# DTUComputeStatisticsAndDataAnalysis/MBPLS

Measured on NVIDIA B200. Metric: MB-PLS NIPALS fit: algorithmic HBM GB/s (n=10k, p=1M, 4 blocks, 20 LV, fp64), higher is better.
Workload: dtype f64

## Files before the change

### mbpls_b200/csrc/fused.cu

```cuda
#include "launch.cuh"
#include "../../include/mbpls_b200.h"

using namespace mbpls;

namespace {

struct FusedArgs {
  const double* Xt;
  double* Xw;
  long ld;
  int n;
  const double* u;
  const double* uu;
  const double* ts;
  const double* rden;
  const double* rden2;
  const int* split_f0;
  const int* split_f1;
  const int* split_block;
  int nsplit;
  int B;
  double* w;
  double* norm_part;
  double* Tnum;
  long ldt;
  double* P_k;
  double* pss;
  const int* done;
  int sync_mode;
};

template <int TG, int EPTC_, int CPF_, int S_>
struct Cfg {
  static constexpr int kTG = TG, EPTC = EPTC_, CPF = CPF_, S = S_;
  static constexpr int G = 512 / TG, EPT = EPTC_ * CPF_, NW = TG / 32;
  static constexpr int UC = TG * EPTC_;
};

template <int NV, int TG>
__device__ __forceinline__ void worker_sum(double (&v)[NV], double* buf, int g, int warp_in_group, int lane) {
  constexpr int NW = TG / 32;
#pragma unroll
  for (int k = 0; k < NV; ++k) v[k] = warp_sum(v[k]);
  if (lane == 0) {
#pragma unroll
    for (int k = 0; k < NV; ++k) buf[k * NW + warp_in_group] = v[k];
  }
  asm volatile("bar.sync %0, %1;" ::"r"(g + 1), "n"(TG) : "memory");
#pragma unroll
  for (int k = 0; k < NV; ++k) {
    const double2* pr = reinterpret_cast<const double2*>(buf + k * NW);
    if (NW == 2) {
      const double2 p0 = pr[0];
      v[k] = p0.x + p0.y;
    } else {
      double grp[NW >= 4 ? NW / 4 : 1];
#pragma unroll
      for (int q = 0; q < NW / 4; ++q) {
        const double2 p0 = pr[2 * q], p1 = pr[2 * q + 1];
        grp[q] = (p0.x + p0.y) + (p1.x + p1.y);
      }
      double t = grp[0];
      if (NW == 8) t = grp[0] + grp[1];
      if (NW == 16) t = (grp[0] + grp[1]) + (grp[2] + grp[3]);
      v[k] = t;
    }
  }
}

__device__ __forceinline__ unsigned atom_inc_smem(unsigned* p) {
  unsigned old;
  asm volatile("atom.relaxed.cta.shared::cta.add.u32 %0, [%1], 1;" : "=r"(old) : "r"(smem_u32(p)) : "memory");
  return old;
}
__device__ __forceinline__ unsigned atom_inc_smem_acqrel(unsigned* p) {
  unsigned old;
  asm volatile("atom.acq_rel.cta.shared::cta.add.u32 %0, [%1], 1;" : "=r"(old) : "r"(smem_u32(p)) : "memory");
  return old;
}

template <class C>
struct Smem {
  double* vec0;
  double* vec1;
  double* ring;
  uint64_t* full;
  unsigned* cnt;
  double* scratch;
  uint64_t* xbar;
  double* xval;
  __device__ Smem(unsigned char* base, long vlen, int nvec) {
    vec0 = reinterpret_cast<double*>(base);
    vec1 = vec0 + vlen;
    ring = vec0 + static_cast<size_t>(nvec) * vlen;
    full = reinterpret_cast<uint64_t*>(ring + static_cast<size_t>(C::G) * C::S * 2 * C::UC);
    cnt = reinterpret_cast<unsigned*>(full + C::G * C::S);
    scratch = reinterpret_cast<double*>(full + 2 * C::G * C::S);
    xbar = reinterpret_cast<uint64_t*>(scratch + static_cast<size_t>(C::G) * 2 * 3 * C::NW);
    xval = reinterpret_cast<double*>(xbar + 2 * C::G);
  }
  __device__ __forceinline__ double* stage(int g, int s) const { return ring + (static_cast<size_t>(g) * C::S + s) * 2 * C::UC; }
};

template <class C>
size_t fused_smem_bytes(long vlen, int nvec) {
  return static_cast<size_t>(nvec) * vlen * 8 + static_cast<size_t>(C::G) * C::S * C::UC * 16 + static_cast<size_t>(C::G) * C::S * 16 +
         static_cast<size_t>(C::G) * 2 * 3 * C::NW * 8 + static_cast<size_t>(C::G) * 32 + 64;
}

template <class C>
__device__ __forceinline__ void issue_chunk(const double* __restrict__ X, long ld, int units, int g, int s, int f, int c,
                                            const Smem<C>& sm) {
  const int nun = min(C::UC, units - c * C::UC);
  const uint32_t bytes = static_cast<uint32_t>(nun) * 16u;
  uint64_t* fb = &sm.full[g * C::S + s];
  mbar_arrive_expect_tx(fb, bytes);
  bulk_g2s(sm.stage(g, s), X + static_cast<size_t>(f) * ld + static_cast<size_t>(c) * C::UC * 2, bytes, fb);
}

template <class C>
__device__ __forceinline__ void init_sync(const Smem<C>& sm, int sync_mode) {
  if (threadIdx.x == 0) {
    for (int i = 0; i < C::G * C::S; ++i) {
      mbar_init(&sm.full[i], 1);
      if (sync_mode == 2) mbar_init(reinterpret_cast<uint64_t*>(&sm.cnt[2 * i]), C::NW);
      else sm.cnt[2 * i] = 0;
    }
    for (int i = 0; i < 2 * C::G; ++i) mbar_init(&sm.xbar[i], 1);
    fence_barrier_init();
  }
}

template <class C>
__device__ __forceinline__ void prime_ring(const double* __restrict__ X, long ld, int units, int ncf, int g, int f0, int f1,
                                           const Smem<C>& sm) {
  int f = f0, c = 0;
  for (int s = 0; s < C::S && f < f1; ++s) {
    issue_chunk<C>(X, ld, units, g, s, f, c, sm);
    if (++c == ncf) { c = 0; ++f; }
  }
}

template <class C>
__device__ __forceinline__ bool arrive_stage(int g, int s, int lane, const Smem<C>& sm, int sync_mode, uint32_t parity) {
  __syncwarp();
  if (lane != 0) return false;
  unsigned* c = &sm.cnt[2 * (g * C::S + s)];
  if (sync_mode == 2) {
    uint64_t* eb = reinterpret_cast<uint64_t*>(c);
    if (mbar_pending_count(mbar_arrive_state(eb)) != 1u) return false;
    mbar_wait(eb, parity);
    fence_proxy_async_smem();
    return true;
  }
  const unsigned old = sync_mode ? atom_inc_smem_acqrel(c) : atom_inc_smem(c);
  if (old != C::NW - 1) return false;
  *reinterpret_cast<volatile unsigned*>(c) = 0;
  if (sync_mode) fence_proxy_async_smem();
  return true;
}

template <class C>
__device__ __forceinline__ void refill_if_last(bool last, const double* __restrict__ X, long ld, int units, int ncf, int g, int s,
                                               int j, int c, int f1, const Smem<C>& sm) {
  if (last) {
    int c2 = c + C::S, f2 = j;
    while (c2 >= ncf) { c2 -= ncf; ++f2; }
    if (f2 < f1) issue_chunk<C>(X, ld, units, g, s, f2, c2, sm);
  }
}

template <class C>
__device__ __forceinline__ double pair_sum(double own, int g, int tg, uint32_t peer, int& xs, uint32_t& xp, const Smem<C>& sm) {
  uint64_t* bar = &sm.xbar[2 * g + xs];
  double* slot = &sm.xval[2 * g + xs];
  if (tg == 0) {
    mbar_arrive_expect_tx(bar, 8);
    st_async_f64(mapa_shared(smem_u32(slot), peer), own, mapa_shared(smem_u32(bar), peer));
  }
  mbar_wait(bar, (xp >> xs) & 1u);
  const double other = *reinterpret_cast<volatile double*>(slot);
  xp ^= 1u << xs;
  xs ^= 1;
  return own + other;
}

__device__ __forceinline__ double2 nan_to_zero(double2 v) {
  if (isnan(v.x)) v.x = 0.0;
  if (isnan(v.y)) v.y = 0.0;
  return v;
}

struct Geo {
  int units;
  int uoff;
  int nloc;
  int wbase;
  uint32_t peer;
  bool lead;
};
template <class C, bool CL>
__device__ __forceinline__ Geo make_geo(long ld, int n) {
  Geo ge;
  const int total = static_cast<int>(ld >> 1);
  if (CL) {
    const uint32_t r = cluster_ctarank();
    ge.units = total >> 1;
    ge.uoff = static_cast<int>(r) * ge.units;
    ge.wbase = static_cast<int>(blockIdx.x >> 1) * C::G;
    ge.peer = r ^ 1u;
    ge.lead = r == 0;
  } else {
    ge.units = total;
    ge.uoff = 0;
    ge.wbase = static_cast<int>(blockIdx.x) * C::G;
    ge.peer = 0;
    ge.lead = true;
  }
  ge.nloc = max(0, min(2 * ge.units, n - 2 * ge.uoff));
  return ge;
}

template <bool NANMODE, class C, bool CL>
__device__ __forceinline__ void fused_trip_body(const FusedArgs& a, const Smem<C>& sm, const Geo& ge) {
  const long ld = a.ld;
  const int units = ge.units;
  const int ncf = (units + C::UC - 1) / C::UC;
  const int g = threadIdx.x / C::kTG, tg = threadIdx.x % C::kTG;
  const int lane = threadIdx.x & 31, wig = tg >> 5;
  const int wk = ge.wbase + g;
  if (wk >= a.nsplit) return;
  const double* __restrict__ X = a.Xt + 2 * static_cast<size_t>(ge.uoff);
  const int f0 = a.split_f0[wk], f1 = a.split_f1[wk];
  if (tg == 0) prime_ring<C>(X, ld, units, ncf, g, f0, f1, sm);
  const double inv_uu = 1.0 / *a.uu;
  const double2* __restrict__ u2 = reinterpret_cast<const double2*>(sm.vec0);
  double* scratch = sm.scratch + static_cast<size_t>(g) * 2 * 3 * C::NW;
  const int sync_mode = a.sync_mode;

  double2 acc[C::EPT], x[C::EPT];
#pragma unroll
  for (int k = 0; k < C::EPT; ++k) acc[k] = x[k] = make_double2(0.0, 0.0);
  double normsq = 0.0, wj = 0.0;
  int s = 0;
  uint32_t ph = 0;
  int flip = 0;
  int xs = 0;
  uint32_t xp = 0;

  for (int j = f0; j <= f1; ++j) {
    const bool load = j < f1;
    const double rd = (NANMODE && load) ? a.rden[j] : inv_uu;
    double numa = 0.0, numb = 0.0, numc = 0.0, numd = 0.0;
    int s_use = s;
    uint32_t ph_use = ph;

    auto load_chunk = [&](const int c) {
      const bool have = load && c < ncf;
      const double2* __restrict__ xs_ = reinterpret_cast<const double2*>(sm.stage(g, s));
      if (have) {
        mbar_wait(&sm.full[g * C::S + s], ph);
        if (++s == C::S) { s = 0; ph ^= 1u; }
      }
      const bool whole = c + 1 < ncf;
#pragma unroll
      for (int e = 0; e < C::EPTC; ++e) {
        const int l = tg + e * C::kTG, gi = c * C::UC + l, k = c * C::EPTC + e;
        acc[k].x = fma(wj, x[k].x, acc[k].x);
        acc[k].y = fma(wj, x[k].y, acc[k].y);
        double2 xv = make_double2(0.0, 0.0), uv = make_double2(0.0, 0.0);
        if (have && (whole || gi < units)) {
          xv = xs_[l];
          uv = u2[gi];
          if (NANMODE) xv = nan_to_zero(xv);
        }
        if (have) {
          if (e & 1) {
            numc = fma(xv.x, uv.x, numc);
            numd = fma(xv.y, uv.y, numd);
          } else {
            numa = fma(xv.x, uv.x, numa);
            numb = fma(xv.y, uv.y, numb);
          }
        }
        x[k] = xv;
      }
    };
    auto release_chunk = [&](const int c) {
      if (!(load && c < ncf)) return;
      refill_if_last<C>(arrive_stage<C>(g, s_use, lane, sm, sync_mode, ph_use), X, ld, units, ncf, g, s_use, j, c, f1, sm);
      if (++s_use == C::S) { s_use = 0; ph_use ^= 1u; }
    };
#pragma unroll
    for (int c = 0; c < C::CPF; ++c) {
      load_chunk(c);
      release_chunk(c);
    }
    if (!load) break;
    double one[1] = {(numa + numb) + (numc + numd)};
    worker_sum<1, C::kTG>(one, scratch + flip * 3 * C::NW, g, wig, lane);
    flip ^= 1;
    if (CL) one[0] = pair_sum<C>(one[0], g, tg, ge.peer, xs, xp, sm);
    wj = one[0] * rd;
    if (tg == 0 && ge.lead) a.w[j] = wj;
    normsq = fma(wj, wj, normsq);
  }

  double2* tn = reinterpret_cast<double2*>(a.Tnum + static_cast<size_t>(wk) * a.ldt) + ge.uoff;
#pragma unroll
  for (int k = 0; k < C::EPT; ++k) {
    const int gi = (k / C::EPTC) * C::UC + tg + (k % C::EPTC) * C::kTG;
    if (gi < units) tn[gi] = acc[k];
  }
  if (tg == 0 && ge.lead) a.norm_part[static_cast<size_t>(wk) * a.B + a.split_block[wk]] = normsq;
}

template <bool NANMODE, class C, bool CL>
__global__ void __launch_bounds__(512, 1) fused_trip_kernel(const FusedArgs a) {
  if (a.done && *a.done) return;
  extern __shared__ __align__(128) unsigned char smem_raw[];
  const Geo ge = make_geo<C, CL>(a.ld, a.n);
  const Smem<C> sm(smem_raw, 2 * ge.units, 1);
  init_sync<C>(sm, a.sync_mode);
  for (int i = threadIdx.x; i < 2 * ge.units; i += blockDim.x) sm.vec0[i] = i < ge.nloc ? a.u[2 * ge.uoff + i] : 0.0;
  __syncthreads();
  if (CL) cluster_sync_all();
  fused_trip_body<NANMODE, C, CL>(a, sm, ge);
  if (CL) cluster_sync_all();
}

template <bool NANMODE, class C, bool CL>
__device__ __forceinline__ void fused_deflate_body(const FusedArgs& a, const Smem<C>& sm, const Geo& ge) {
  const long ld = a.ld;
  const int units = ge.units;
  const int ncf = (units + C::UC - 1) / C::UC;
  const bool next = a.u != nullptr;
  const int g = threadIdx.x / C::kTG, tg = threadIdx.x % C::kTG;
  const int lane = threadIdx.x & 31, wig = tg >> 5;
  const int wk = ge.wbase + g;
  if (wk >= a.nsplit) return;
  double* __restrict__ X = a.Xw + 2 * static_cast<size_t>(ge.uoff);
  const int f0 = a.split_f0[wk], f1 = a.split_f1[wk];
  if (tg == 0) prime_ring<C>(X, ld, units, ncf, g, f0, f1, sm);
  const double inv_uu = next ? 1.0 / *a.uu : 1.0;
  const double2* __restrict__ ts2 = reinterpret_cast<const double2*>(sm.vec0);
  const double2* __restrict__ u2 = reinterpret_cast<const double2*>(sm.vec1);
  double* scratch = sm.scratch + static_cast<size_t>(g) * 2 * 3 * C::NW;
  const double qnan = __longlong_as_double(0x7ff8000000000000LL);
  const int sync_mode = a.sync_mode;

  double2 acc[C::EPT], x[C::EPT];
#pragma unroll
  for (int k = 0; k < C::EPT; ++k) acc[k] = x[k] = make_double2(0.0, 0.0);
  double normsq = 0.0, wj = 0.0;
  int s = 0;
  uint32_t ph = 0;
  int flip = 0;
  int xs = 0;
  uint32_t xp = 0;

  for (int j = f0; j <= f1; ++j) {
    const bool load = j < f1;
    const double rdp = (NANMODE && load) ? a.rden[j] : 1.0;
    const double rdw = (NANMODE && load && next) ? a.rden2[j] : inv_uu;
    double pa = 0.0, pb = 0.0, pc = 0.0, pd = 0.0;
    uint32_t mx = 0, my = 0;
    int s_use = s;
    uint32_t ph_use = ph;

    auto load_chunk = [&](const int c) {
      const bool have = load && c < ncf;
      const double2* __restrict__ xs_ = reinterpret_cast<const double2*>(sm.stage(g, s));
      if (have) {
        mbar_wait(&sm.full[g * C::S + s], ph);
        if (++s == C::S) { s = 0; ph ^= 1u; }
      }
      const bool whole = c + 1 < ncf;
#pragma unroll
      for (int e = 0; e < C::EPTC; ++e) {
        const int l = tg + e * C::kTG, gi = c * C::UC + l, k = c * C::EPTC + e;
        acc[k].x = fma(wj, x[k].x, acc[k].x);
        acc[k].y = fma(wj, x[k].y, acc[k].y);
        double2 xv = make_double2(0.0, 0.0), tv = make_double2(0.0, 0.0);
        if (have && (whole || gi < units)) {
          xv = xs_[l];
          tv = ts2[gi];
          if (NANMODE) {
            if (isnan(xv.x)) { xv.x = 0.0; mx |= 1u << k; }
            if (isnan(xv.y)) { xv.y = 0.0; my |= 1u << k; }
          }
        }
        if (e & 1) {
          pc = fma(xv.x, tv.x, pc);
          pd = fma(xv.y, tv.y, pd);
        } else {
          pa = fma(xv.x, tv.x, pa);
          pb = fma(xv.y, tv.y, pb);
        }
        x[k] = xv;
      }
    };
    auto release_chunk = [&](const int c) {
      if (!(load && c < ncf)) return;
      refill_if_last<C>(arrive_stage<C>(g, s_use, lane, sm, sync_mode, ph_use), X, ld, units, ncf, g, s_use, j, c, f1, sm);
      if (++s_use == C::S) { s_use = 0; ph_use ^= 1u; }
    };
#pragma unroll
    for (int c = 0; c < C::CPF; ++c) {
      load_chunk(c);
      release_chunk(c);
    }
    if (!load) break;
    double one[1] = {(pa + pb) + (pc + pd)};
    worker_sum<1, C::kTG>(one, scratch + flip * 3 * C::NW, g, wig, lane);
    flip ^= 1;
    if (CL) one[0] = pair_sum<C>(one[0], g, tg, ge.peer, xs, xp, sm);
    const double pj = one[0] * rdp;
    double2* __restrict__ xg = reinterpret_cast<double2*>(X + static_cast<size_t>(j) * ld);
    double wa = 0.0, wb = 0.0, wc = 0.0, wd = 0.0;
#pragma unroll
    for (int k = 0; k < C::EPT; ++k) {
      const int gi = (k / C::EPTC) * C::UC + tg + (k % C::EPTC) * C::kTG;
      if (((k / C::EPTC) + 1 < ncf) || gi < units) {
        const double2 tv = ts2[gi];
        const double2 uv = u2[gi];
        double2 xn;
        xn.x = __dsub_rn(x[k].x, __dmul_rn(tv.x, pj));
        xn.y = __dsub_rn(x[k].y, __dmul_rn(tv.y, pj));
        if (NANMODE) {
          double2 out = xn;
          if ((mx >> k) & 1u) { out.x = qnan; xn.x = 0.0; }
          if ((my >> k) & 1u) { out.y = qnan; xn.y = 0.0; }
          st_stream(xg + gi, out);
        } else {
          st_stream(xg + gi, xn);
        }
        x[k] = xn;
        if (next) {
          if (k & 1) {
            wc = fma(xn.x, uv.x, wc);
            wd = fma(xn.y, uv.y, wd);
          } else {
            wa = fma(xn.x, uv.x, wa);
            wb = fma(xn.y, uv.y, wb);
          }
        }
      }
    }
    if (next) {
      double two[1] = {(wa + wb) + (wc + wd)};
      worker_sum<1, C::kTG>(two, scratch + flip * 3 * C::NW, g, wig, lane);
      flip ^= 1;
      if (CL) two[0] = pair_sum<C>(two[0], g, tg, ge.peer, xs, xp, sm);
      wj = two[0] * rdw;
      normsq = fma(wj, wj, normsq);
    }
    if (tg == 0 && ge.lead) {
      a.P_k[j] = pj;
      a.pss[j] = pj * pj;
      if (next) a.w[j] = wj;
    }
  }
  if (!next) return;
  double2* tn = reinterpret_cast<double2*>(a.Tnum + static_cast<size_t>(wk) * a.ldt) + ge.uoff;
#pragma unroll
  for (int k = 0; k < C::EPT; ++k) {
    const int gi = (k / C::EPTC) * C::UC + tg + (k % C::EPTC) * C::kTG;
    if (gi < units) tn[gi] = acc[k];
  }
  if (tg == 0 && ge.lead) a.norm_part[static_cast<size_t>(wk) * a.B + a.split_block[wk]] = normsq;
}

template <bool NANMODE, class C, bool CL>
__global__ void __launch_bounds__(512, 1) fused_deflate_kernel(const FusedArgs a) {
  if (a.done && !*a.done) return;
  extern __shared__ __align__(128) unsigned char smem_raw[];
  const Geo ge = make_geo<C, CL>(a.ld, a.n);
  const Smem<C> sm(smem_raw, 2 * ge.units, 2);
  init_sync<C>(sm, a.sync_mode);
  const bool next = a.u != nullptr;
  for (int i = threadIdx.x; i < 2 * ge.units; i += blockDim.x) {
    sm.vec0[i] = i < ge.nloc ? a.ts[2 * ge.uoff + i] : 0.0;
    sm.vec1[i] = (next && i < ge.nloc) ? a.u[2 * ge.uoff + i] : 0.0;
  }
  __syncthreads();
  if (CL) cluster_sync_all();
  fused_deflate_body<NANMODE, C, CL>(a, sm, ge);
  if (CL) cluster_sync_all();
}

struct StdArgs {
  double* mean;
  double* var;
  double* scale;
  long long* seen;
  double* zss;
};

template <class C>
__global__ void __launch_bounds__(512, 1) fused_standardize_kernel(const FusedArgs a, const StdArgs so) {
  extern __shared__ __align__(128) unsigned char smem_raw[];
  const Geo ge = make_geo<C, false>(a.ld, a.n);
  const Smem<C> sm(smem_raw, 2 * ge.units, 1);
  init_sync<C>(sm, a.sync_mode);
  for (int i = threadIdx.x; i < 2 * ge.units; i += blockDim.x) sm.vec0[i] = i < a.n ? a.u[i] : 0.0;
  __syncthreads();
  const long ld = a.ld;
  const int units = ge.units;
  const int ncf = (units + C::UC - 1) / C::UC;
  const int g = threadIdx.x / C::kTG, tg = threadIdx.x % C::kTG;
  const int lane = threadIdx.x & 31, wig = tg >> 5;
  const int wk = ge.wbase + g;
  if (wk >= a.nsplit) return;
  double* __restrict__ X = a.Xw;
  const int f0 = a.split_f0[wk], f1 = a.split_f1[wk];
  if (tg == 0) prime_ring<C>(X, ld, units, ncf, g, f0, f1, sm);
  const double inv_uu = 1.0 / *a.uu;
  const double cnt = static_cast<double>(a.n);
  const double2* __restrict__ u2 = reinterpret_cast<const double2*>(sm.vec0);
  double* scratch = sm.scratch + static_cast<size_t>(g) * 2 * 3 * C::NW;
  const int sync_mode = a.sync_mode;
  const int nn = a.n;
  double2 acc[C::EPT], x[C::EPT];
#pragma unroll
  for (int k = 0; k < C::EPT; ++k) acc[k] = x[k] = make_double2(0.0, 0.0);
  double normsq = 0.0, wj = 0.0;
  int s = 0;
  uint32_t ph = 0;
  int flip = 0;

  for (int j = f0; j <= f1; ++j) {
    const bool load = j < f1;
    double sa = 0.0, sb = 0.0, sc = 0.0, sd = 0.0;
    int s_use = s;
    uint32_t ph_use = ph;
#pragma unroll
    for (int c = 0; c < C::CPF; ++c) {
      const bool have = load && c < ncf;
      const double2* __restrict__ xs_ = reinterpret_cast<const double2*>(sm.stage(g, s));
      if (have) {
        mbar_wait(&sm.full[g * C::S + s], ph);
        if (++s == C::S) { s = 0; ph ^= 1u; }
      }
      const bool whole = c + 1 < ncf;
#pragma unroll
      for (int e = 0; e < C::EPTC; ++e) {
        const int l = tg + e * C::kTG, gi = c * C::UC + l, k = c * C::EPTC + e;
        acc[k].x = fma(wj, x[k].x, acc[k].x);
        acc[k].y = fma(wj, x[k].y, acc[k].y);
        double2 xv = make_double2(0.0, 0.0);
        if (have && (whole || gi < units)) xv = xs_[l];
        if (e & 1) {
          sc += xv.x;
          sd += xv.y;
        } else {
          sa += xv.x;
          sb += xv.y;
        }
        x[k] = xv;
      }
      if (have) {
        refill_if_last<C>(arrive_stage<C>(g, s_use, lane, sm, sync_mode, ph_use), X, ld, units, ncf, g, s_use, j, c, f1, sm);
        if (++s_use == C::S) { s_use = 0; ph_use ^= 1u; }
      }
    }
    if (!load) break;
    double one[1] = {(sa + sb) + (sc + sd)};
    worker_sum<1, C::kTG>(one, scratch + flip * 3 * C::NW, g, wig, lane);
    flip ^= 1;
    const double mean = one[0] / cnt;
    double thr[3] = {0.0, 0.0, 0.0};
#pragma unroll
    for (int k = 0; k < C::EPT; ++k) {
      const int gi = (k / C::EPTC) * C::UC + tg + (k % C::EPTC) * C::kTG;
      const int e0 = 2 * gi;
      double2 d;
      d.x = e0 < nn ? x[k].x - mean : 0.0;
      d.y = e0 + 1 < nn ? x[k].y - mean : 0.0;
      if (e0 < nn) {
        const double2 uv = u2[gi];
        thr[2] = fma(d.x, uv.x, thr[2]);
        thr[2] = fma(d.y, uv.y, thr[2]);
      }
      thr[0] += d.x + d.y;
      thr[1] = fma(d.x, d.x, thr[1]);
      thr[1] = fma(d.y, d.y, thr[1]);
      x[k] = d;
    }
    worker_sum<3, C::kTG>(thr, scratch + flip * 3 * C::NW, g, wig, lane);
    flip ^= 1;
    const double var = (thr[1] - thr[0] * thr[0] / cnt) / cnt;
    const double eps = 2.220446049250313e-16;
    const double bound = cnt * eps * var + (cnt * mean * eps) * (cnt * mean * eps);
    const double scale = (var <= bound) ? 1.0 : sqrt(var);
    wj = thr[2] / scale * inv_uu;
    normsq = fma(wj, wj, normsq);
    double2* __restrict__ xg = reinterpret_cast<double2*>(X + static_cast<size_t>(j) * ld);
    const UniformDivisor by_scale(scale);
#pragma unroll
    for (int k = 0; k < C::EPT; ++k) {
      const int gi = (k / C::EPTC) * C::UC + tg + (k % C::EPTC) * C::kTG;
      if (((k / C::EPTC) + 1 < ncf) || gi < units) {
        double2 z;
        z.x = by_scale(x[k].x);
        z.y = by_scale(x[k].y);
        st_stream(xg + gi, z);
        x[k] = z;
      }
    }
    if (tg == 0) {
      so.mean[j] = mean;
      so.var[j] = var;
      so.scale[j] = scale;
      so.seen[j] = static_cast<long long>(a.n);
      so.zss[j] = thr[1] / (scale * scale);
      a.w[j] = wj;
    }
  }
  double2* tn = reinterpret_cast<double2*>(a.Tnum + static_cast<size_t>(wk) * a.ldt);
#pragma unroll
  for (int k = 0; k < C::EPT; ++k) {
    const int gi = (k / C::EPTC) * C::UC + tg + (k % C::EPTC) * C::kTG;
    if (gi < units) tn[gi] = acc[k];
  }
  if (tg == 0) a.norm_part[static_cast<size_t>(wk) * a.B + a.split_block[wk]] = normsq;
}

using CfgA = Cfg<512, 5, 2, 3>;
using CfgA4 = Cfg<512, 2, 5, 4>;
using CfgB = Cfg<256, 5, 2, 3>;
using CfgC = Cfg<128, 5, 2, 4>;
using CfgD = Cfg<64, 10, 1, 2>;

int env_int(const char* name, int dflt) {
  const char* e = getenv(name);
  return e ? atoi(e) : dflt;
}
bool cluster_enabled() {
  static int v = -1;
  if (v < 0) v = env_int("MBPLS_FUSED_CLUSTER", 1) != 0;
  return v != 0;
}
int default_sync_mode() {
  static int v = -1;
  if (v < 0) {
    v = env_int("MBPLS_FUSED_SYNC", 2);
    if (v < 0 || v > 2) v = 2;
  }
  return v;
}

template <class K>
int launch_fused(K kernel, const FusedArgs& a, int workers_per_cta, size_t smem, bool cluster, cudaStream_t st) {
  if (smem > static_cast<size_t>(smem_optin())) return MBPLS_ERR_SIZE;
  cudaFuncSetAttribute(kernel, cudaFuncAttributeMaxDynamicSharedMemorySize, static_cast<int>(smem));
  const int groups = (a.nsplit + workers_per_cta - 1) / workers_per_cta;
  cudaLaunchConfig_t cfg = {};
  cfg.gridDim = dim3(static_cast<unsigned>(cluster ? 2 * groups : groups), 1, 1);
  cfg.blockDim = dim3(512, 1, 1);
  cfg.dynamicSmemBytes = smem;
  cfg.stream = st;
  cudaLaunchAttribute attr[1];
  attr[0].id = cudaLaunchAttributeClusterDimension;
  attr[0].val.clusterDim.x = 2;
  attr[0].val.clusterDim.y = 1;
  attr[0].val.clusterDim.z = 1;
  cfg.attrs = attr;
  cfg.numAttrs = cluster ? 1 : 0;
  const cudaError_t e = cudaLaunchKernelEx(&cfg, kernel, a);
  return e == cudaSuccess ? MBPLS_OK : MBPLS_CUDA_ERR(e);
}

template <class K>
int max_active_pairs(K kernel, size_t smem) {
  if (cudaFuncSetAttribute(kernel, cudaFuncAttributeMaxDynamicSharedMemorySize, static_cast<int>(smem)) != cudaSuccess) {
    cudaGetLastError();
    return 0;
  }
  cudaLaunchConfig_t cfg = {};
  cfg.gridDim = dim3(static_cast<unsigned>(num_sms() / 2 * 2), 1, 1);
  cfg.blockDim = dim3(512, 1, 1);
  cfg.dynamicSmemBytes = smem;
  cudaLaunchAttribute attr[1];
  attr[0].id = cudaLaunchAttributeClusterDimension;
  attr[0].val.clusterDim.x = 2;
  attr[0].val.clusterDim.y = 1;
  attr[0].val.clusterDim.z = 1;
  cfg.attrs = attr;
  cfg.numAttrs = 1;
  int n = 0;
  if (cudaOccupancyMaxActiveClusters(&n, kernel, &cfg) != cudaSuccess) {
    cudaGetLastError();
    return 0;
  }
  return n;
}

struct Plan {
  int trip = 0, deflate = 0;
  bool trip_cl = false, deflate_cl = false;
  int workers = 0;
};

Plan plan_of(long ld) {
  Plan pl;
  if (ld < 16 || (ld % 16) != 0) return pl;
  const long units = ld >> 1;
  const int sms = num_sms();
  if (units <= 640) { pl.trip = pl.deflate = 4; pl.workers = sms * CfgD::G; return pl; }
  if (units <= 1280) { pl.trip = pl.deflate = 3; pl.workers = sms * CfgC::G; return pl; }
  if (units <= 2560) { pl.trip = pl.deflate = 2; pl.workers = sms * CfgB::G; return pl; }
  static int pairs_b = -1, pairs_a = -1, pairs_a4 = -1;
  if (units <= 5120) {
    pl.trip = 1;
    pl.deflate = 5;
    pl.workers = sms * CfgA::G;
    if (cluster_enabled()) {
      if (pairs_b < 0) pairs_b = max_active_pairs(fused_deflate_kernel<false, CfgB, true>, fused_smem_bytes<CfgB>(ld >> 1, 2));
      if (pairs_b * CfgB::G >= pl.workers * 9 / 10) {
        pl.deflate = 2;
        pl.deflate_cl = true;
        pl.workers = min(pl.workers, pairs_b * CfgB::G);
      }
    }
    return pl;
  }
  if (units <= 10240 && cluster_enabled()) {
    if (pairs_a < 0) pairs_a = max_active_pairs(fused_trip_kernel<false, CfgA, true>, fused_smem_bytes<CfgA>(ld >> 1, 1));
    if (pairs_a4 < 0) pairs_a4 = max_active_pairs(fused_deflate_kernel<false, CfgA4, true>, fused_smem_bytes<CfgA4>(ld >> 1, 2));
    const int pairs = min(pairs_a, pairs_a4);
    if (pairs > 0) {
      pl.trip = 1;
      pl.deflate = 5;
      pl.trip_cl = pl.deflate_cl = true;
      pl.workers = pairs * CfgA::G;
    }
  }
  return pl;
}

template <bool NANMODE, bool CL>
int dispatch_trip(int cfg, const FusedArgs& a, cudaStream_t st) {
  const long vlen = CL ? a.ld >> 1 : a.ld;
  switch (cfg) {
    case 1: return launch_fused(fused_trip_kernel<NANMODE, CfgA, CL>, a, CfgA::G, fused_smem_bytes<CfgA>(vlen, 1), CL, st);
    case 2: return launch_fused(fused_trip_kernel<NANMODE, CfgB, CL>, a, CfgB::G, fused_smem_bytes<CfgB>(vlen, 1), CL, st);
    case 3: return launch_fused(fused_trip_kernel<NANMODE, CfgC, false>, a, CfgC::G, fused_smem_bytes<CfgC>(a.ld, 1), false, st);
    case 4: return launch_fused(fused_trip_kernel<NANMODE, CfgD, false>, a, CfgD::G, fused_smem_bytes<CfgD>(a.ld, 1), false, st);
    default: return MBPLS_ERR_SIZE;
  }
}

template <bool NANMODE, bool CL>
int dispatch_deflate(int cfg, const FusedArgs& a, cudaStream_t st) {
  const long vlen = CL ? a.ld >> 1 : a.ld;
  switch (cfg) {
    case 5: return launch_fused(fused_deflate_kernel<NANMODE, CfgA4, CL>, a, CfgA4::G, fused_smem_bytes<CfgA4>(vlen, 2), CL, st);
    case 2: return launch_fused(fused_deflate_kernel<NANMODE, CfgB, CL>, a, CfgB::G, fused_smem_bytes<CfgB>(vlen, 2), CL, st);
    case 3: return launch_fused(fused_deflate_kernel<NANMODE, CfgC, false>, a, CfgC::G, fused_smem_bytes<CfgC>(a.ld, 2), false, st);
    case 4: return launch_fused(fused_deflate_kernel<NANMODE, CfgD, false>, a, CfgD::G, fused_smem_bytes<CfgD>(a.ld, 2), false, st);
    default: return MBPLS_ERR_SIZE;
  }
}

}

extern "C" {

int mbpls_fused_workers_per_sm_pair(long ld) {
  if (ld < 16 || (ld % 16) != 0) return 0;
  const long units = ld >> 1;
  return units <= 640 ? 16 : units <= 1280 ? 8 : units <= 2560 ? 4 : units <= 5120 ? 2 : units <= 10240 ? 1 : 0;
}

int mbpls_fused_total_workers(long ld) { return plan_of(ld).workers; }

int mbpls_fused_uses_clusters(long ld) {
  const Plan pl = plan_of(ld);
  return (pl.trip_cl ? 1 : 0) | (pl.deflate_cl ? 2 : 0);
}

int mbpls_nipals_fused_trip_f64(const double* Xt, long ld, int n, const double* u, const double* uu, const double* rden,
                                const int* split_f0, const int* split_f1, const int* split_block, int nsplit, int B, double* w,
                                double* norm_part, double* Tnum, long ldt, const int* done, void* stream) {
  if (!Xt || !u || !uu || !split_f0 || !split_f1 || !split_block || !w || !norm_part || !Tnum || ld < n || ldt < ld || B < 1)
    return MBPLS_ERR_ARG;
  if (nsplit == 0) return MBPLS_OK;
  const Plan pl = plan_of(ld);
  if (!pl.trip || nsplit > pl.workers) return MBPLS_ERR_SIZE;
  FusedArgs a{Xt, nullptr, ld, n, u, uu, nullptr, rden, nullptr, split_f0, split_f1, split_block, nsplit, B,
              w, norm_part, Tnum, ldt, nullptr, nullptr, done, default_sync_mode()};
  cudaStream_t st = static_cast<cudaStream_t>(stream);
  if (pl.trip_cl) return rden ? dispatch_trip<true, true>(pl.trip, a, st) : dispatch_trip<false, true>(pl.trip, a, st);
  return rden ? dispatch_trip<true, false>(pl.trip, a, st) : dispatch_trip<false, false>(pl.trip, a, st);
}

int mbpls_fused_deflate_f64(double* Xt, long ld, int n, const double* ts, const double* rden_ts, const double* u0,
                            const double* u0u0, const double* rden_u0, const int* split_f0, const int* split_f1,
                            const int* split_block, int nsplit, int B, double* P_k, double* pss, double* w_next, double* norm_part,
                            double* Tnum, long ldt, const int* only_if_done, void* stream) {
  if (!Xt || !ts || !split_f0 || !split_f1 || !split_block || !P_k || !pss || ld < n || B < 1) return MBPLS_ERR_ARG;
  if (u0 && (!u0u0 || !w_next || !norm_part || !Tnum || ldt < ld || (rden_ts && !rden_u0))) return MBPLS_ERR_ARG;
  if (nsplit == 0) return MBPLS_OK;
  const Plan pl = plan_of(ld);
  if (!pl.deflate || nsplit > pl.workers) return MBPLS_ERR_SIZE;
  FusedArgs a{nullptr, Xt, ld, n, u0, u0u0, ts, rden_ts, rden_u0, split_f0, split_f1, split_block, nsplit, B,
              w_next, norm_part, Tnum, ldt, P_k, pss, only_if_done, default_sync_mode()};
  cudaStream_t st = static_cast<cudaStream_t>(stream);
  if (pl.deflate_cl) return rden_ts ? dispatch_deflate<true, true>(pl.deflate, a, st) : dispatch_deflate<false, true>(pl.deflate, a, st);
  return rden_ts ? dispatch_deflate<true, false>(pl.deflate, a, st) : dispatch_deflate<false, false>(pl.deflate, a, st);
}

int mbpls_fused_standardize_f64(double* Xt, long ld, int n, const double* u0, const double* u0u0, const int* split_f0,
                                const int* split_f1, const int* split_block, int nsplit, int B, double* mean, double* var,
                                double* scale, long long* seen, double* zss, double* w, double* norm_part, double* Tnum, long ldt,
                                void* stream) {
  if (!Xt || !u0 || !u0u0 || !split_f0 || !split_f1 || !split_block || !mean || !var || !scale || !seen || !zss || !w ||
      !norm_part || !Tnum || ld < n || ldt < ld || B < 1)
    return MBPLS_ERR_ARG;
  if (nsplit == 0) return MBPLS_OK;
  const Plan pl = plan_of(ld);
  if (!pl.trip || pl.trip_cl || nsplit > pl.workers) return MBPLS_ERR_SIZE;
  FusedArgs a{nullptr, Xt, ld, n, u0, u0u0, nullptr, nullptr, nullptr, split_f0, split_f1, split_block, nsplit, B,
              w, norm_part, Tnum, ldt, nullptr, nullptr, nullptr, default_sync_mode()};
  const StdArgs so{mean, var, scale, seen, zss};
  cudaStream_t st = static_cast<cudaStream_t>(stream);
#define STD_LAUNCH(CFG)                                                                                                      \
  do {                                                                                                                       \
    const size_t smem = fused_smem_bytes<CFG>(ld, 1);                                                                        \
    if (smem > static_cast<size_t>(smem_optin())) return MBPLS_ERR_SIZE;                                                     \
    cudaFuncSetAttribute(fused_standardize_kernel<CFG>, cudaFuncAttributeMaxDynamicSharedMemorySize, static_cast<int>(smem)); \
    fused_standardize_kernel<CFG><<<(nsplit + CFG::G - 1) / CFG::G, 512, smem, st>>>(a, so);                                  \
  } while (0)
  switch (pl.trip) {
    case 1: STD_LAUNCH(CfgA); break;
    case 2: STD_LAUNCH(CfgB); break;
    case 3: STD_LAUNCH(CfgC); break;
    case 4: STD_LAUNCH(CfgD); break;
    default: return MBPLS_ERR_SIZE;
  }
#undef STD_LAUNCH
  MBPLS_RETURN_LAST();
}

}
```

Before: 11540.

## Stage score vector u in tensor memory instead of shared memory in trip kernel

The trip kernel now allocates Blackwell tensor memory (tcgen05.alloc) and stores each thread's slice of u there, reading it back with tcgen05.ld inside the inner loop instead of from shared memory. This removes the u vector from the shared-memory footprint, which shrinks the dynamic smem request and may let more CTAs or larger rings fit. It also cuts shared-memory bandwidth pressure alongside the bulk-copy ring. In exchange it adds tcgen05 ld/wait latency per unit, alloc/dealloc and fence overhead, and relies on the per-thread layout fitting 256 columns.

```diff
diff --git a/mbpls_b200/csrc/fused.cu b/mbpls_b200/csrc/fused.cu
--- a/mbpls_b200/csrc/fused.cu
+++ b/mbpls_b200/csrc/fused.cu
@@ -89,6 +89,7 @@
   double* scratch;
   uint64_t* xbar;
   double* xval;
+  uint32_t* tslot;
   __device__ Smem(unsigned char* base, long vlen, int nvec) {
     vec0 = reinterpret_cast<double*>(base);
     vec1 = vec0 + vlen;
@@ -98,6 +99,7 @@
     scratch = reinterpret_cast<double*>(full + 2 * C::G * C::S);
     xbar = reinterpret_cast<uint64_t*>(scratch + static_cast<size_t>(C::G) * 2 * 3 * C::NW);
     xval = reinterpret_cast<double*>(xbar + 2 * C::G);
+    tslot = reinterpret_cast<uint32_t*>(xval + 2 * C::G);
   }
   __device__ __forceinline__ double* stage(int g, int s) const { return ring + (static_cast<size_t>(g) * C::S + s) * 2 * C::UC; }
 };
@@ -107,6 +109,49 @@
   return static_cast<size_t>(nvec) * vlen * 8 + static_cast<size_t>(C::G) * C::S * C::UC * 16 + static_cast<size_t>(C::G) * C::S * 16 +
          static_cast<size_t>(C::G) * 2 * 3 * C::NW * 8 + static_cast<size_t>(C::G) * 32 + 64;
 }
+
+__device__ __forceinline__ void tmem_fence_before() { asm volatile("tcgen05.fence::before_thread_sync;" ::: "memory"); }
+__device__ __forceinline__ void tmem_fence_after() { asm volatile("tcgen05.fence::after_thread_sync;" ::: "memory"); }
+template <int NCOLS>
+__device__ __forceinline__ void tmem_alloc(uint32_t* slot) {
+  asm volatile("tcgen05.alloc.cta_group::1.sync.aligned.shared::cta.b32 [%0], %1;" ::"r"(smem_u32(slot)), "n"(NCOLS) : "memory");
+  asm volatile("tcgen05.relinquish_alloc_permit.cta_group::1.sync.aligned;" ::: "memory");
+}
+template <int NCOLS>
+__device__ __forceinline__ void tmem_dealloc(uint32_t base) {
+  asm volatile("tcgen05.dealloc.cta_group::1.sync.aligned.b32 %0, %1;" ::"r"(base), "n"(NCOLS) : "memory");
+}
+__device__ __forceinline__ uint32_t tmem_thread_base(uint32_t base, int cols) {
+  const int warp = threadIdx.x >> 5;
+  return base + (static_cast<uint32_t>((warp & 3) * 32) << 16) + static_cast<uint32_t>((warp >> 2) * cols);
+}
+__device__ __forceinline__ void tmem_st_unit(uint32_t taddr, double2 v) {
+  asm volatile("tcgen05.st.sync.aligned.32x32b.x4.b32 [%0], {%1, %2, %3, %4};" ::"r"(taddr), "r"(__double2loint(v.x)),
+               "r"(__double2hiint(v.x)), "r"(__double2loint(v.y)), "r"(__double2hiint(v.y))
+               : "memory");
+}
+__device__ __forceinline__ void tmem_ld_unit(uint32_t taddr, uint32_t (&r)[4]) {
+  asm volatile("tcgen05.ld.sync.aligned.32x32b.x4.b32 {%0, %1, %2, %3}, [%4];" : "=r"(r[0]), "=r"(r[1]), "=r"(r[2]), "=r"(r[3]) : "r"(taddr));
+}
+__device__ __forceinline__ void tmem_wait_ld() { asm volatile("tcgen05.wait::ld.sync.aligned;" ::: "memory"); }
+__device__ __forceinline__ double2 tmem_unit(uint32_t (&r)[4]) {
+  asm volatile("" : "+r"(r[0]), "+r"(r[1]), "+r"(r[2]), "+r"(r[3]));
+  return make_double2(__hiloint2double(r[1], r[0]), __hiloint2double(r[3], r[2]));
+}
+template <class C, int STRIDE>
+__device__ __forceinline__ void tmem_fill(uint32_t taddr, const double* src, int uoff, int nloc) {
+  const int tg = threadIdx.x % C::kTG;
+#pragma unroll
+  for (int k = 0; k < C::EPT; ++k) {
+    const int i = 2 * ((k / C::EPTC) * C::UC + tg + (k % C::EPTC) * C::kTG);
+    double2 v = make_double2(0.0, 0.0);
+    if (src && i < nloc) v.x = src[2 * uoff + i];
+    if (src && i + 1 < nloc) v.y = src[2 * uoff + i + 1];
+    tmem_st_unit(taddr + k * STRIDE, v);
+  }
+  asm volatile("tcgen05.wait::st.sync.aligned;" ::: "memory");
+}
+constexpr int kTripCols = 256;
 
 template <class C>
 __device__ __forceinline__ void issue_chunk(const double* __restrict__ X, long ld, int units, int g, int s, int f, int c,
@@ -222,7 +267,7 @@
 }
 
 template <bool NANMODE, class C, bool CL>
-__device__ __forceinline__ void fused_trip_body(const FusedArgs& a, const Smem<C>& sm, const Geo& ge) {
+__device__ __forceinline__ void fused_trip_body(const FusedArgs& a, const Smem<C>& sm, const Geo& ge, uint32_t tm) {
   const long ld = a.ld;
   const int units = ge.units;
   const int ncf = (units + C::UC - 1) / C::UC;
@@ -234,7 +279,6 @@
   const int f0 = a.split_f0[wk], f1 = a.split_f1[wk];
   if (tg == 0) prime_ring<C>(X, ld, units, ncf, g, f0, f1, sm);
   const double inv_uu = 1.0 / *a.uu;
-  const double2* __restrict__ u2 = reinterpret_cast<const double2*>(sm.vec0);
   double* scratch = sm.scratch + static_cast<size_t>(g) * 2 * 3 * C::NW;
   const int sync_mode = a.sync_mode;
 
@@ -266,15 +310,18 @@
 #pragma unroll
       for (int e = 0; e < C::EPTC; ++e) {
         const int l = tg + e * C::kTG, gi = c * C::UC + l, k = c * C::EPTC + e;
+        uint32_t ur[4];
+        if (have) tmem_ld_unit(tm + 4 * k, ur);
         acc[k].x = fma(wj, x[k].x, acc[k].x);
         acc[k].y = fma(wj, x[k].y, acc[k].y);
-        double2 xv = make_double2(0.0, 0.0), uv = make_double2(0.0, 0.0);
+        double2 xv = make_double2(0.0, 0.0);
         if (have && (whole || gi < units)) {
           xv = xs_[l];
-          uv = u2[gi];
           if (NANMODE) xv = nan_to_zero(xv);
         }
         if (have) {
+          tmem_wait_ld();
+          const double2 uv = tmem_unit(ur);
           if (e & 1) {
             numc = fma(xv.x, uv.x, numc);
             numd = fma(xv.y, uv.y, numd);
@@ -320,13 +367,22 @@
   if (a.done && *a.done) return;
   extern __shared__ __align__(128) unsigned char smem_raw[];
   const Geo ge = make_geo<C, CL>(a.ld, a.n);
-  const Smem<C> sm(smem_raw, 2 * ge.units, 1);
+  static_assert(4 * 4 * C::EPT <= kTripCols, "u does not fit the TMEM allocation");
+  const Smem<C> sm(smem_raw, 0, 0);
+  if (threadIdx.x < 32) tmem_alloc<kTripCols>(sm.tslot);
   init_sync<C>(sm, a.sync_mode);
-  for (int i = threadIdx.x; i < 2 * ge.units; i += blockDim.x) sm.vec0[i] = i < ge.nloc ? a.u[2 * ge.uoff + i] : 0.0;
+  tmem_fence_before();
   __syncthreads();
+  tmem_fence_after();
+  const uint32_t tm = tmem_thread_base(*sm.tslot, 4 * C::EPT);
+  tmem_fill<C, 4>(tm, a.u, ge.uoff, ge.nloc);
   if (CL) cluster_sync_all();
-  fused_trip_body<NANMODE, C, CL>(a, sm, ge);
+  fused_trip_body<NANMODE, C, CL>(a, sm, ge, tm);
+  tmem_fence_before();
   if (CL) cluster_sync_all();
+  else __syncthreads();
+  tmem_fence_after();
+  if (threadIdx.x < 32) tmem_dealloc<kTripCols>(*sm.tslot);
 }
 
 template <bool NANMODE, class C, bool CL>
@@ -726,7 +782,7 @@
     return pl;
   }
   if (units <= 10240 && cluster_enabled()) {
-    if (pairs_a < 0) pairs_a = max_active_pairs(fused_trip_kernel<false, CfgA, true>, fused_smem_bytes<CfgA>(ld >> 1, 1));
+    if (pairs_a < 0) pairs_a = max_active_pairs(fused_trip_kernel<false, CfgA, true>, fused_smem_bytes<CfgA>(0, 0));
     if (pairs_a4 < 0) pairs_a4 = max_active_pairs(fused_deflate_kernel<false, CfgA4, true>, fused_smem_bytes<CfgA4>(ld >> 1, 2));
     const int pairs = min(pairs_a, pairs_a4);
     if (pairs > 0) {
@@ -741,12 +797,11 @@
 
 template <bool NANMODE, bool CL>
 int dispatch_trip(int cfg, const FusedArgs& a, cudaStream_t st) {
-  const long vlen = CL ? a.ld >> 1 : a.ld;
   switch (cfg) {
-    case 1: return launch_fused(fused_trip_kernel<NANMODE, CfgA, CL>, a, CfgA::G, fused_smem_bytes<CfgA>(vlen, 1), CL, st);
-    case 2: return launch_fused(fused_trip_kernel<NANMODE, CfgB, CL>, a, CfgB::G, fused_smem_bytes<CfgB>(vlen, 1), CL, st);
-    case 3: return launch_fused(fused_trip_kernel<NANMODE, CfgC, false>, a, CfgC::G, fused_smem_bytes<CfgC>(a.ld, 1), false, st);
-    case 4: return launch_fused(fused_trip_kernel<NANMODE, CfgD, false>, a, CfgD::G, fused_smem_bytes<CfgD>(a.ld, 1), false, st);
+    case 1: return launch_fused(fused_trip_kernel<NANMODE, CfgA, CL>, a, CfgA::G, fused_smem_bytes<CfgA>(0, 0), CL, st);
+    case 2: return launch_fused(fused_trip_kernel<NANMODE, CfgB, CL>, a, CfgB::G, fused_smem_bytes<CfgB>(0, 0), CL, st);
+    case 3: return launch_fused(fused_trip_kernel<NANMODE, CfgC, false>, a, CfgC::G, fused_smem_bytes<CfgC>(0, 0), false, st);
+    case 4: return launch_fused(fused_trip_kernel<NANMODE, CfgD, false>, a, CfgD::G, fused_smem_bytes<CfgD>(0, 0), false, st);
     default: return MBPLS_ERR_SIZE;
   }
 }
```

New measurement: 11550 (median of 6 runs). About the same (+0.1%).

## Add TMA-pipelined 2-CTA cluster trip kernel for mid-size rows

Applied to the files above, without the earlier changes.

Adds a trip kernel for row lengths up to 5120 units in which a pair of 256-thread CTAs splits each row. A 4D tensor map plus bulk copies stream rows into a 5-stage mbarrier-guarded shared-memory ring. Per-row dot products are reduced across the pair with async DSMEM stores, and the w-weighted accumulation into Tnum is done in registers. It aims to raise HBM streaming efficiency with deeper async prefetch and less per-row synchronisation. In exchange it adds tensor-map encoding on every call and depends on cluster occupancy.

```diff
diff --git a/mbpls_b200/csrc/fused.cu b/mbpls_b200/csrc/fused.cu
--- a/mbpls_b200/csrc/fused.cu
+++ b/mbpls_b200/csrc/fused.cu
@@ -1,3 +1,5 @@
+#include <cuda.h>
+#include <cudaTypedefs.h>
 #include "launch.cuh"
 #include "../../include/mbpls_b200.h"
 
@@ -327,6 +329,206 @@
   if (CL) cluster_sync_all();
   fused_trip_body<NANMODE, C, CL>(a, sm, ge);
   if (CL) cluster_sync_all();
+}
+
+constexpr int kPT = 256;
+constexpr int kPM = 10;
+constexpr int kPS = 5;
+constexpr int kPSU = kPT * kPM;
+
+size_t trip_pair_smem_bytes() { return static_cast<size_t>(kPS) * kPSU * 16 + (2 * kPS + 2) * 8 + 2 * 16 * 8; }
+
+struct SplitCursor {
+  int si, j, f1;
+  __device__ __forceinline__ void seek(const FusedArgs& a, int P) {
+    while (si < a.nsplit) {
+      j = a.split_f0[si];
+      f1 = a.split_f1[si];
+      if (j < f1) return;
+      si += P;
+    }
+  }
+  __device__ __forceinline__ bool live(const FusedArgs& a) const { return si < a.nsplit; }
+  __device__ __forceinline__ void next(const FusedArgs& a, int P) {
+    if (live(a) && ++j == f1) {
+      si += P;
+      seek(a, P);
+    }
+  }
+};
+
+__device__ __forceinline__ int pair_copy_units(int units, int m, uint32_t r) {
+  return max(0, min(256, units - 512 * m - 256 * static_cast<int>(r)));
+}
+
+__device__ __forceinline__ void issue_pair_stage(const FusedArgs& a, const CUtensorMap* tm, int f, int units, uint32_t r,
+                                                 double2* stage, uint64_t* fb, uint32_t tx) {
+  mbar_arrive_expect_tx(fb, tx);
+  asm volatile(
+      "cp.async.bulk.tensor.4d.shared::cluster.global.tile.mbarrier::complete_tx::bytes [%0], [%1, {%2, %3, %4, %5}], [%6];" ::"r"(
+          smem_u32(stage)),
+      "l"(reinterpret_cast<uint64_t>(tm)), "r"(0), "r"(2 * static_cast<int>(r)), "r"(0), "r"(f), "r"(smem_u32(fb))
+      : "memory");
+  const int G = units / 512;
+  const int cnt = G < kPM ? pair_copy_units(units, G, r) : 0;
+  if (cnt > 0)
+    bulk_g2s(stage + 256 * G, a.Xt + static_cast<size_t>(f) * a.ld + 1024 * G + 512 * static_cast<int>(r),
+             static_cast<uint32_t>(cnt) * 16u, fb);
+}
+
+template <bool NANMODE>
+__global__ void __launch_bounds__(kPT, 1) fused_trip_pair_kernel(const FusedArgs a, const __grid_constant__ CUtensorMap tmap) {
+  if (a.done && *a.done) return;
+  extern __shared__ __align__(128) unsigned char smem_raw[];
+  double2* ring = reinterpret_cast<double2*>(smem_raw);
+  uint64_t* full = reinterpret_cast<uint64_t*>(ring + kPS * kPSU);
+  uint64_t* empty = full + kPS;
+  uint64_t* xbar = empty + kPS;
+  double* xval = reinterpret_cast<double*>(xbar + 2);
+  const uint32_t r = cluster_ctarank(), peer = r ^ 1u;
+  const int t = threadIdx.x, lane = t & 31, warp = t >> 5;
+  const int c0 = static_cast<int>(blockIdx.x >> 1), P = static_cast<int>(gridDim.x >> 1);
+  const int units = static_cast<int>(a.ld >> 1);
+  const int base = 256 * static_cast<int>(r) + t;
+  uint32_t tx = 0;
+#pragma unroll
+  for (int m = 0; m < kPM; ++m) tx += static_cast<uint32_t>(pair_copy_units(units, m, r)) * 16u;
+
+  if (t == 0) {
+    for (int i = 0; i < kPS; ++i) {
+      mbar_init(&full[i], 1);
+      mbar_init(&empty[i], kPT / 32);
+    }
+    for (int i = 0; i < 2; ++i) mbar_init(&xbar[i], kPT / 32);
+    fence_barrier_init();
+  }
+  for (int i = t; i < kPS * kPSU; i += kPT) {
+    const int l = i % kPSU;
+    if (l % 256 >= pair_copy_units(units, l / 256, r)) ring[i] = make_double2(0.0, 0.0);
+  }
+  double2 u[kPM];
+#pragma unroll
+  for (int m = 0; m < kPM; ++m) {
+    const int i0 = 2 * (512 * m + base);
+    u[m] = make_double2(i0 < a.n ? a.u[i0] : 0.0, i0 + 1 < a.n ? a.u[i0 + 1] : 0.0);
+  }
+  for (int si = c0; si < a.nsplit; si += P) {
+    if (a.split_f0[si] < a.split_f1[si]) continue;
+    double2* tn = reinterpret_cast<double2*>(a.Tnum + static_cast<size_t>(si) * a.ldt);
+#pragma unroll
+    for (int m = 0; m < kPM; ++m)
+      if (512 * m + base < units) tn[512 * m + base] = make_double2(0.0, 0.0);
+    if (t == 0 && r == 0) a.norm_part[static_cast<size_t>(si) * a.B + a.split_block[si]] = 0.0;
+  }
+  __syncthreads();
+  cluster_sync_all();
+
+  SplitCursor cons{c0, 0, 0}, iss{c0, 0, 0};
+  cons.seek(a, P);
+  iss.seek(a, P);
+  for (int s = 0; s < kPS; ++s) {
+    if (t == 0 && iss.live(a)) issue_pair_stage(a, &tmap, iss.j, units, r, ring + s * kPSU, &full[s], tx);
+    iss.next(a, P);
+  }
+
+  const double inv_uu = 1.0 / *a.uu;
+  double2 acc[kPM], xa[kPM], xb[kPM];
+#pragma unroll
+  for (int m = 0; m < kPM; ++m) acc[m] = xa[m] = xb[m] = make_double2(0.0, 0.0);
+  double normsq = 0.0;
+  int s = 0;
+  uint32_t ph = 0;
+  int qpub = 0, qwait = 0;
+
+  auto load = [&](double2 (&x)[kPM]) -> double {
+    mbar_wait(&full[s], ph);
+    const double2* st = ring + s * kPSU + t;
+    double numa = 0.0, numb = 0.0, numc = 0.0, numd = 0.0;
+#pragma unroll
+    for (int m = 0; m < kPM; ++m) {
+      double2 v = st[256 * m];
+      if (NANMODE) v = nan_to_zero(v);
+      if ((m % 5) & 1) {
+        numc = fma(v.x, u[m].x, numc);
+        numd = fma(v.y, u[m].y, numd);
+      } else {
+        numa = fma(v.x, u[m].x, numa);
+        numb = fma(v.y, u[m].y, numb);
+      }
+      x[m] = v;
+    }
+    __syncwarp();
+    if (lane == 0 && mbar_pending_count(mbar_arrive_state(&empty[s])) == 1u) {
+      mbar_wait(&empty[s], ph);
+      fence_proxy_async_smem();
+      if (iss.live(a)) issue_pair_stage(a, &tmap, iss.j, units, r, ring + s * kPSU, &full[s], tx);
+    }
+    iss.next(a, P);
+    if (++s == kPS) {
+      s = 0;
+      ph ^= 1u;
+    }
+    return warp_sum((numa + numb) + (numc + numd));
+  };
+  auto publish = [&](double v) {
+    __syncwarp();
+    if (lane == 0) {
+      const int sl = qpub & 1;
+      double* dst = xval + 16 * sl + 8 * static_cast<int>(r) + warp;
+      *dst = v;
+      st_async_f64(mapa_shared(smem_u32(dst), peer), v, mapa_shared(smem_u32(&xbar[sl]), peer));
+      if (warp == 0) mbar_arrive_expect_tx(&xbar[sl], 8 * (kPT / 32));
+      else mbar_arrive(&xbar[sl]);
+    }
+    ++qpub;
+  };
+  auto reduce = [&]() -> double {
+    const int sl = qwait & 1;
+    mbar_wait(&xbar[sl], (qwait >> 1) & 1);
+    const double2* pr = reinterpret_cast<const double2*>(xval + 16 * sl);
+    double grp[4];
+#pragma unroll
+    for (int q = 0; q < 4; ++q) {
+      const double2 p0 = pr[2 * q], p1 = pr[2 * q + 1];
+      grp[q] = (p0.x + p0.y) + (p1.x + p1.y);
+    }
+    ++qwait;
+    return (grp[0] + grp[1]) + (grp[2] + grp[3]);
+  };
+  auto step = [&](double2 (&cur)[kPM], double2 (&nxt)[kPM]) -> bool {
+    const SplitCursor pend = cons;
+    cons.next(a, P);
+    const bool more = cons.live(a);
+    const double rd = NANMODE ? a.rden[pend.j] : inv_uu;
+    const double v = more ? load(nxt) : 0.0;
+    const double wj = reduce() * rd;
+    if (t == 0 && r == 0) a.w[pend.j] = wj;
+    normsq = fma(wj, wj, normsq);
+#pragma unroll
+    for (int m = 0; m < kPM; ++m) {
+      acc[m].x = fma(wj, cur[m].x, acc[m].x);
+      acc[m].y = fma(wj, cur[m].y, acc[m].y);
+    }
+    if (pend.j + 1 == pend.f1) {
+      double2* tn = reinterpret_cast<double2*>(a.Tnum + static_cast<size_t>(pend.si) * a.ldt);
+#pragma unroll
+      for (int m = 0; m < kPM; ++m) {
+        if (512 * m + base < units) tn[512 * m + base] = acc[m];
+        acc[m] = make_double2(0.0, 0.0);
+      }
+      if (t == 0 && r == 0) a.norm_part[static_cast<size_t>(pend.si) * a.B + a.split_block[pend.si]] = normsq;
+      normsq = 0.0;
+    }
+    if (more) publish(v);
+    return more;
+  };
+
+  if (cons.live(a)) {
+    publish(load(xa));
+    while (step(xa, xb) && step(xb, xa)) {
+    }
+  }
+  cluster_sync_all();
 }
 
 template <bool NANMODE, class C, bool CL>
@@ -672,14 +874,14 @@
 }
 
 template <class K>
-int max_active_pairs(K kernel, size_t smem) {
+int max_active_pairs(K kernel, size_t smem, int threads = 512) {
   if (cudaFuncSetAttribute(kernel, cudaFuncAttributeMaxDynamicSharedMemorySize, static_cast<int>(smem)) != cudaSuccess) {
     cudaGetLastError();
     return 0;
   }
   cudaLaunchConfig_t cfg = {};
   cfg.gridDim = dim3(static_cast<unsigned>(num_sms() / 2 * 2), 1, 1);
-  cfg.blockDim = dim3(512, 1, 1);
+  cfg.blockDim = dim3(static_cast<unsigned>(threads), 1, 1);
   cfg.dynamicSmemBytes = smem;
   cudaLaunchAttribute attr[1];
   attr[0].id = cudaLaunchAttributeClusterDimension;
@@ -700,7 +902,10 @@
   int trip = 0, deflate = 0;
   bool trip_cl = false, deflate_cl = false;
   int workers = 0;
+  int trip_pairs = 0;
 };
+
+bool trip_pairs_enabled() { return env_int("MBPLS_TRIP_PAIRS", 1) != 0; }
 
 Plan plan_of(long ld) {
   Plan pl;
@@ -710,7 +915,7 @@
   if (units <= 640) { pl.trip = pl.deflate = 4; pl.workers = sms * CfgD::G; return pl; }
   if (units <= 1280) { pl.trip = pl.deflate = 3; pl.workers = sms * CfgC::G; return pl; }
   if (units <= 2560) { pl.trip = pl.deflate = 2; pl.workers = sms * CfgB::G; return pl; }
-  static int pairs_b = -1, pairs_a = -1, pairs_a4 = -1;
+  static int pairs_b = -1, pairs_a = -1, pairs_a4 = -1, pairs_t = -1;
   if (units <= 5120) {
     pl.trip = 1;
     pl.deflate = 5;
@@ -723,6 +928,10 @@
         pl.workers = min(pl.workers, pairs_b * CfgB::G);
       }
     }
+    if (trip_pairs_enabled()) {
+      if (pairs_t < 0) pairs_t = max_active_pairs(fused_trip_pair_kernel<false>, trip_pair_smem_bytes(), kPT);
+      if (2 * pairs_t >= pl.workers) pl.trip_pairs = pairs_t;
+    }
     return pl;
   }
   if (units <= 10240 && cluster_enabled()) {
@@ -749,6 +958,51 @@
     case 4: return launch_fused(fused_trip_kernel<NANMODE, CfgD, false>, a, CfgD::G, fused_smem_bytes<CfgD>(a.ld, 1), false, st);
     default: return MBPLS_ERR_SIZE;
   }
+}
+
+bool make_pair_tmap(CUtensorMap* tm, const double* Xt, long ld) {
+  static PFN_cuTensorMapEncodeTiled encode = nullptr;
+  if (!encode) {
+    void* fn = nullptr;
+    cudaDriverEntryPointQueryResult q;
+    if (cudaGetDriverEntryPoint("cuTensorMapEncodeTiled", &fn, cudaEnableDefault, &q) != cudaSuccess ||
+        q != cudaDriverEntryPointSuccess || !fn) {
+      cudaGetLastError();
+      return false;
+    }
+    encode = reinterpret_cast<PFN_cuTensorMapEncodeTiled>(fn);
+  }
+  const cuuint32_t G = static_cast<cuuint32_t>((ld >> 1) / 512);
+  const cuuint64_t dim[4] = {256, 4, G, 1u << 30};
+  const cuuint64_t stride[3] = {2048, 8192, static_cast<cuuint64_t>(ld) * 8};
+  const cuuint32_t box[4] = {256, 2, G, 1};
+  const cuuint32_t estr[4] = {1, 1, 1, 1};
+  return encode(tm, CU_TENSOR_MAP_DATA_TYPE_FLOAT64, 4, const_cast<double*>(Xt), dim, stride, box, estr,
+                CU_TENSOR_MAP_INTERLEAVE_NONE, CU_TENSOR_MAP_SWIZZLE_NONE, static_cast<CUtensorMapL2promotion>(env_int("MBPLS_PAIR_L2P", 3)),
+                CU_TENSOR_MAP_FLOAT_OOB_FILL_NONE) == CUDA_SUCCESS;
+}
+
+template <bool NANMODE>
+int launch_trip_pairs(const FusedArgs& a, int pairs, cudaStream_t st) {
+  const size_t smem = trip_pair_smem_bytes();
+  if (smem > static_cast<size_t>(smem_optin())) return MBPLS_ERR_SIZE;
+  CUtensorMap tm;
+  if (!make_pair_tmap(&tm, a.Xt, a.ld)) return MBPLS_ERR_ARG;
+  cudaFuncSetAttribute(fused_trip_pair_kernel<NANMODE>, cudaFuncAttributeMaxDynamicSharedMemorySize, static_cast<int>(smem));
+  cudaLaunchConfig_t cfg = {};
+  cfg.gridDim = dim3(static_cast<unsigned>(2 * min(pairs, a.nsplit)), 1, 1);
+  cfg.blockDim = dim3(kPT, 1, 1);
+  cfg.dynamicSmemBytes = smem;
+  cfg.stream = st;
+  cudaLaunchAttribute attr[1];
+  attr[0].id = cudaLaunchAttributeClusterDimension;
+  attr[0].val.clusterDim.x = 2;
+  attr[0].val.clusterDim.y = 1;
+  attr[0].val.clusterDim.z = 1;
+  cfg.attrs = attr;
+  cfg.numAttrs = 1;
+  const cudaError_t e = cudaLaunchKernelEx(&cfg, fused_trip_pair_kernel<NANMODE>, a, tm);
+  return e == cudaSuccess ? MBPLS_OK : MBPLS_CUDA_ERR(e);
 }
 
 template <bool NANMODE, bool CL>
@@ -791,6 +1045,8 @@
   FusedArgs a{Xt, nullptr, ld, n, u, uu, nullptr, rden, nullptr, split_f0, split_f1, split_block, nsplit, B,
               w, norm_part, Tnum, ldt, nullptr, nullptr, done, default_sync_mode()};
   cudaStream_t st = static_cast<cudaStream_t>(stream);
+  if (pl.trip_pairs) a.sync_mode = env_int("MBPLS_PAIR_DEBUG", 0);
+  if (pl.trip_pairs) return rden ? launch_trip_pairs<true>(a, pl.trip_pairs, st) : launch_trip_pairs<false>(a, pl.trip_pairs, st);
   if (pl.trip_cl) return rden ? dispatch_trip<true, true>(pl.trip, a, st) : dispatch_trip<false, true>(pl.trip, a, st);
   return rden ? dispatch_trip<true, false>(pl.trip, a, st) : dispatch_trip<false, false>(pl.trip, a, st);
 }
```

Measured after the change: 11560 before, 11790 after (median of 6 runs). 1.02x the previous value.
